# locuslab/lcp-physics

Hardware: AMD Instinct MI355X
Metric: sim steps/sec at batch=4096x16 contacts, fwd+bwd (higher is better)
Workload: dtype f64; 1 GPU; configs[2]: batch=4096 x 16 contacts (4-box stack, 4 pts/interface; nz 15, nineq 64, neq 3) per GPU, fp32 I/O, LCP forward + backward (implicit diff), mode=fused, bwd=dense; step outputs: new_v and the moved pose (engines.py:76-77, bodies.py:80-82), multipliers kept in the workspace in fp64; launch=eager: one ctypes call per kernel launch, device_spin_up_steps=4100, nonzero_status=0, global_batch=4096, parallelism=scenes sharded x1, no collectives, control_plane=single process

## Files before the change

lcp_physics_amd/csrc/lcp_quad_kernels.inc:

```
#pragma once
#include "lcp_quad_prims.h"

#ifndef LCP_Q_LAUNDER_IN_PLACE
#define LCP_Q_LAUNDER_IN_PLACE 1
#endif
#ifndef LCP_Q_PEEL_INIT
#define LCP_Q_PEEL_INIT 1
#endif
#ifndef LCP_Q_UNROLL_PASS
#define LCP_Q_UNROLL_PASS 1
#endif
#ifndef LCP_Q_NT_STORES
#define LCP_Q_NT_STORES 0
#endif
#ifndef LCP_Q_EXP_SPW
#define LCP_Q_EXP_SPW 4
#endif
#ifndef LCP_Q_RCP_STEP
#define LCP_Q_RCP_STEP 1
#endif
#ifndef LCP_Q_STEP_FAST
#define LCP_Q_STEP_FAST 1
#endif
#ifndef LCP_Q_OCC2
#define LCP_Q_OCC2 1
#endif
#ifndef LCP_Q_ROWL
#define LCP_Q_ROWL 0
#endif
#ifndef LCP_Q_BEST_LDS
#define LCP_Q_BEST_LDS 1
#endif

namespace lcp {
namespace q16 {

template <typename TI, typename TC>
struct LdsQ {
  TI* GL;
  TI* GTL;
  TI* AtL;
  TC* GAL;
  TC* S11;
// ... 331 lines not shown
  oz = m4<TC>(-wz.n, -wz.f1, -wz.f2, -wz.g);
  if (!valid) oz = m4<TC>(0, 0, 0, 0);
  os = m4<TC>((-rs.n - oz.n) * di.n, (-rs.f1 - oz.f1) * di.f1, (-rs.f2 - oz.f2) * di.f2, (-rs.g - oz.g) * di.g);
  if (!valid) os = m4<TC>(0, 0, 0, 0);
  oy = dy;
  const XV<TC, XH> gw = S.Gtw(oz.n, oz.f1 - oz.f2);
  XV<TC, XH> g1;
  static_for<XH>([&](auto HX) LCP_INL { g1.v[HX] = -rx.v[HX] - gw.v[HX]; });
  if (S.e > 0) { const XV<TC, XH> ay = S.Aty(dy); static_for<XH>([&](auto HX) LCP_INL { g1.v[HX] -= ay.v[HX]; }); }
  static_for<XH>([&](auto HX) LCP_INL { ox.v[HX] = S.qid[HX] * g1.v[HX]; });
  LCP_QTICK(pr, 5)
}

template <typename TC, bool PINC = false, int NZF = 0, int EF = 0, int NCF = 0>
struct PrimQ {
  static constexpr int NZF_ = NZF, EF_ = EF, NCF_ = NCF;
  static constexpr bool TRIM_ = PINC && NZF > 0;
  static constexpr int CLO_ = TRIM_ ? EF : 0, CHI_ = TRIM_ ? NZF : 16;
  TC idn, i1, i2, kap;
  TC udx, ude;
  bool pin_rt;
  __device__ __forceinline__ bool pin() const { return PINC || pin_rt; }
  TC sp[EQ];
};
template <typename TI, typename TC, typename PQ, typename SQ>
__device__ __forceinline__ M4<TC> minv_pq(const PQ& R, const SQ& S, const M4<TC>& t) {
  M4<TC> o;
  o.n = R.idn * t.n;
  o.g = R.kap * ((t.g - S.mu * o.n) + fma(R.i1, t.f1, R.i2 * t.f2));
  o.f1 = R.i1 * (t.f1 - o.g);
  o.f2 = R.i2 * (t.f2 - o.g);
  return o;
}
template <typename TI, typename TC, typename PQ, typename SQ>
__device__ __forceinline__ bool factor_pq(TC (&xr)[20], TC (&er)[20], PQ& R, const SQ& S, const M4<TC>& D,
                                          bool valid LCP_QPROF_ARG) {
  const int l16 = launder(S.l16), ncw = PQ::NCF_ > 0 ? PQ::NCF_ : __builtin_amdgcn_readfirstlane(S.ncw);
  const int nz = PQ::NZF_ > 0 ? PQ::NZF_ : __builtin_amdgcn_readfirstlane(S.nz), e = PQ::NZF_ > 0 ? PQ::EF_ : __builtin_amdgcn_readfirstlane(S.e);
  R.idn = fast_rcp(D.n); R.i1 = fast_rcp(D.f1); R.i2 = fast_rcp(D.f2);
  R.kap = fast_rcp(D.g + (R.i1 + R.i2));
  const TC b00 = valid ? R.idn : (TC)0;
  const TC b10 = valid ? R.kap * (R.i1 - R.i2) * (S.mu * R.idn) : (TC)0;
  const TC b11 = valid ? R.kap * fma(R.i1 + R.i2, D.g, (TC)4 * (R.i1 * R.i2)) : (TC)0;
  TC p0[16], p1[16];
  const int oz = lds_opaque_zero();
  constexpr int CLO = PQ::CLO_, CHI = PQ::CHI_;
  static_for<CHI - CLO>([&](auto Jq) LCP_INL {
    constexpr int J = CLO + Jq;
    const TC c = (TC)S.template jcv<J>(oz), t = (TC)S.template jtv<J>(oz); p0[J] = b00 * c; p1[J] = fma(b10, c, b11 * t);
  });
  {
    const TI* at = S.L.AtL + oz;
    const TC dsel = (l16 < nz) ? S.qd[0] : (TC)1;
    static_for<CHI - CLO>([&](auto Jq) LCP_INL { constexpr int J = CLO + Jq; xr[J] = (l16 == J) ? dsel : (TC)0; });
    if (!R.pin()) {
      static_for<16>([&](auto J) LCP_INL { er[J] = (l16 < EQ) ? (TC)at[(l16 & (EQ - 1)) * 16 + J] : (TC)0; });
      static_for<EQ>([&](auto A) LCP_INL {
        xr[16 + A] = (TC)at[A * 16 + l16];
        er[16 + A] = (l16 == A && A >= e) ? (TC)1 : (TC)0;
      });
    }
  }
  {
    const TI* gl = S.L.GL + l16 + oz;
    const TI* gtl = S.L.GTL + l16 + oz;
    static_for<2>([&](auto Hh) LCP_INL {
      constexpr int C0 = 8 * Hh;
      if (C0 < ncw) {
        TI gv[8], tv[8];
        if constexpr (sizeof(S.gcol) == sizeof(TC)) {
          static_for<8>([&](auto I) LCP_INL { gv[I] = gl[(C0 + I) * 16]; tv[I] = gtl[(C0 + I) * 16]; });
          __builtin_amdgcn_sched_barrier(0);
        }
        static_for<8>([&](auto I) LCP_INL {
          constexpr int C = C0 + I;
          TC a, b;
          if constexpr (sizeof(S.gcol) == sizeof(TC)) { a = (TC)gv[I]; b = (TC)tv[I]; } else { a = S.gcol[C]; b = S.tcol[C]; }
          if constexpr (PQ::TRIM_) {
            constexpr int NA = (CHI < 8 ? CHI : 8) - CLO, NB = CHI > 8 ? CHI - 8 : 0;
            pq_formN<C, CLO, (NA > 0 ? NA : 0)>(xr, p0, p1, a, b);
            pq_formN<C, 8, NB>(xr, p0, p1, a, b);
          } else {
            pq_form8<C, 0>(xr, p0, p1, a, b);
            pq_form8<C, 8>(xr, p0, p1, a, b);
          }
        });
      }
    });
  }
  LCP_QTICK(pr, 1)
  bool singular = false;
  R.udx = 1; R.ude = 1;
  if (R.pin()) {
    TC pivv = bc<0>(xr[0]);
    TC inv = (TC)1;
    bool primed = false;
    static_for<16>([&](auto K) LCP_INL {
      constexpr int k = K;
      if (k >= e && k < nz) {
        if (!primed) { pivv = bc<k>(xr[k]); inv = fast_rcp(pivv); primed = true; }
        singular = singular || (pivv == (TC)0);
        const TC sk = xr[k] * inv;
        const TC lx = keep_if(sk, l16 > k);
        xr[k] = (l16 == k) ? xr[k] : sk;
        R.udx = (l16 == k) ? inv : R.udx;
        if constexpr (k + 1 < 16) {
          fnmac_bc<k>(xr[k + 1], xr[k + 1], lx);
          pivv = bc<(k + 1) & 15>(xr[k + 1]); inv = fast_rcp(pivv);
          lu_cols_x<k, k + 2, 14 - k>(xr, lx);
        }
      }
    });
    if constexpr (!PQ::TRIM_)
      static_for<EQ>([&](auto A_) LCP_INL { constexpr int a = A_; R.sp[a] = xr[a]; xr[a] = (a < e) ? (TC)0 : xr[a]; });
    LCP_QTICK(pr, 2)
    return singular;
  }
  TC pivv = bc<0>(xr[0]);
  TC inv = fast_rcp(pivv);
  static_for<16>([&](auto K) LCP_INL {
    constexpr int k = K;
    if (k < nz) {
      singular = singular || (pivv == (TC)0);
      const TC lx = (l16 > k) ? xr[k] * inv : (TC)0;
      const TC le = er[k] * inv;
      xr[k] = (l16 > k) ? lx : xr[k];
      er[k] = le;
      R.udx = (l16 == k) ? inv : R.udx;
      fnmac_bc<k>(er[k + 1], xr[k + 1], le);
      fnmac_bc<k>(xr[k + 1], xr[k + 1], lx);
      if constexpr (k + 1 < 16) { pivv = bc<(k + 1) & 15>(xr[k + 1]); inv = fast_rcp(pivv); }
      lu_cols_p<k, k + 2, 18 - k>(xr, er, lx, le);
    }
  });
  static_for<EQ>([&](auto A_) LCP_INL {
    constexpr int a = A_, k = 16 + A_;
    if (a < e) {
      const TC pivv = bc<a>(er[k]);
      singular = singular || (pivv == (TC)0);
      const TC inv = fast_rcp(pivv);
      const TC le = (l16 > a) ? er[k] * inv : (TC)0;
      er[k] = (l16 > a) ? le : er[k];
      R.ude = (l16 == a) ? inv : R.ude;
      static_for<EQ - 1 - a>([&](auto JJ) LCP_INL { constexpr int j = k + 1 + JJ; fnmac_bc<a>(er[j], er[j], le); });
    }
  });
  LCP_QTICK(pr, 2)
  return singular;
}

template <typename TI, typename TC, typename PQ, typename SQ>
__device__ __forceinline__ void solve_kkt_pq(const SQ& S, const TC (&xr)[20], const TC (&er)[20], const PQ& R,
                                             const M4<TC>& di, bool valid, const XV<TC, 1>& rx, const M4<TC>& rs, const M4<TC>& rz, TC ry,
                                             XV<TC, 1>& ox, M4<TC>& os, M4<TC>& oz, TC& oy LCP_QPROF_ARG) {
  const int l16 = S.l16;
  const int nz = PQ::NZF_ > 0 ? PQ::NZF_ : __builtin_amdgcn_readfirstlane(S.nz), e = PQ::NZF_ > 0 ? PQ::EF_ : __builtin_amdgcn_readfirstlane(S.e);
  M4<TC> q = m4<TC>(rs.n * di.n - rz.n, rs.f1 * di.f1 - rz.f1, rs.f2 * di.f2 - rz.f2, rs.g * di.g - rz.g);
  if (!valid) q = m4<TC>(0, 0, 0, 0);
  const M4<TC> u = minv_pq<TI, TC, PQ, SQ>(R, S, q);
  const XV<TC, 1> gu = S.template Gtw<true>(valid ? u.n : (TC)0, valid ? u.f1 - u.f2 : (TC)0);
  TC wx = (l16 < nz) ? gu.v[0] - rx.v[0] : (TC)0;
  TC we = (l16 < e) ? -ry : (TC)0;
  LCP_QTICK(pr, 3)
  if (R.pin()) {
    if constexpr (PQ::TRIM_) {
      static_for<PQ::CHI_ - PQ::CLO_>([&](auto Kq) LCP_INL { constexpr int k = PQ::CLO_ + Kq; fnmac_bc<k>(wx, wx, keep_if(xr[k], l16 > k)); });
      static_for<PQ::CHI_ - PQ::CLO_>([&](auto KR) LCP_INL { constexpr int k = PQ::CHI_ - 1 - KR; fnmac_bc<k>(wx, wx, keep_if(xr[k], l16 < k)); });
    } else {
    if (e > 0) static_for<EQ>([&](auto A_) LCP_INL { constexpr int a = A_; fnmac_bc<a>(wx, we, keep_if(R.sp[a], a < e)); });
    static_for<4>([&](auto Gq) LCP_INL {
      if (4 * Gq < nz) static_for<4>([&](auto Kq) LCP_INL {
        constexpr int k = 4 * Gq + Kq;
        fnmac_bc<k>(wx, wx, keep_if(xr[k], l16 > k));
      });
    });
    static_for<4>([&](auto GR) LCP_INL {
      constexpr int Gq = 3 - GR;
      if (4 * Gq < nz) static_for<4>([&](auto KR) LCP_INL {
        constexpr int k = 4 * Gq + 3 - KR;
        fnmac_bc<k>(wx, wx, keep_if(xr[k], l16 < k));
      });
    });
    }
    LCP_QTICK(pr, 4)
    ox.v[0] = (l16 < e) ? we : ((l16 < nz) ? wx * R.udx : (TC)0);
    oy = (l16 < e) ? wx : (TC)0;
    TC gn, gt;
    S.template Gv<true, PQ::CLO_, PQ::CHI_>(ox, gn, gt);
    oz = minv_pq<TI, TC, PQ, SQ>(R, S, m4<TC>(gn - q.n, gt - q.f1, -gt - q.f2, -q.g));
    if (!valid) oz = m4<TC>(0, 0, 0, 0);
    os = m4<TC>((-rs.n - oz.n) * di.n, (-rs.f1 - oz.f1) * di.f1, (-rs.f2 - oz.f2) * di.f2, (-rs.g - oz.g) * di.g);
    if (!valid) os = m4<TC>(0, 0, 0, 0);
    LCP_QTICK(pr, 5)
    return;
  }
  static_for<4>([&](auto Gq) LCP_INL {
    if (4 * Gq < nz) static_for<4>([&](auto Kq) LCP_INL {
      constexpr int k = 4 * Gq + Kq;
      fnmac_bc<k>(we, wx, er[k]);
      fnmac_bc<k>(wx, wx, keep_if(xr[k], l16 > k));
    });
  });
  if (e > 0) {
    static_for<EQ>([&](auto A_) LCP_INL { constexpr int a = A_; fnmac_bc<a>(we, we, keep_if(er[16 + a], l16 > a)); });
    static_for<EQ>([&](auto AR) LCP_INL {
      constexpr int a = EQ - 1 - AR;
      const TC xs = we * R.ude;
      fnmac_bc<a>(wx, xs, xr[16 + a]);
      fnmac_bc<a>(we, xs, keep_if(er[16 + a], l16 < a));
    });
  }
  static_for<4>([&](auto GR) LCP_INL {
    constexpr int Gq = 3 - GR;
    if (4 * Gq < nz) static_for<4>([&](auto KR) LCP_INL {
      constexpr int k = 4 * Gq + 3 - KR;
      const TC xs = wx * R.udx;
      fnmac_bc<k>(wx, xs, keep_if(xr[k], l16 < k));
    });
  });
  LCP_QTICK(pr, 4)
  ox.v[0] = (l16 < nz) ? wx * R.udx : (TC)0;
  oy = (l16 < e) ? we * R.ude : (TC)0;
  TC gn, gt;
  S.template Gv<true>(ox, gn, gt);
  oz = minv_pq<TI, TC, PQ, SQ>(R, S, m4<TC>(gn - q.n, gt - q.f1, -gt - q.f2, -q.g));
  if (!valid) oz = m4<TC>(0, 0, 0, 0);
  os = m4<TC>((-rs.n - oz.n) * di.n, (-rs.f1 - oz.f1) * di.f1, (-rs.f2 - oz.f2) * di.f2, (-rs.g - oz.g) * di.g);
  if (!valid) os = m4<TC>(0, 0, 0, 0);
  LCP_QTICK(pr, 5)
}

template <typename TC>
__device__ __forceinline__ TC step_pair_q(const M4<TC>& z, const M4<TC>& dz, const M4<TC>& s, const M4<TC>& ds, bool valid) {
  const TC ninf = -inf_of<TC>(), pinf = inf_of<TC>();
  const M4<TC> az = m4<TC>(qdiv_x(-z.n, dz.n), qdiv_x(-z.f1, dz.f1), qdiv_x(-z.f2, dz.f2), qdiv_x(-z.g, dz.g));
  const M4<TC> as = m4<TC>(qdiv_x(-s.n, ds.n), qdiv_x(-s.f1, ds.f1), qdiv_x(-s.f2, ds.f2), qdiv_x(-s.g, ds.g));
  auto key4 = [&](const M4<TC>& a) { return umax(umax(nan_key(a.n), nan_key(a.f1)), umax(nan_key(a.f2), nan_key(a.g))); };
#if LCP_Q_STEP_FAST
  {
    const bool oz = !(dz.n > (TC)0) || !(dz.f1 > (TC)0) || !(dz.f2 > (TC)0) || !(dz.g > (TC)0);
    const bool os = !(ds.n > (TC)0) || !(ds.f1 > (TC)0) || !(ds.f2 > (TC)0) || !(ds.g > (TC)0);
    const bool nn = key_is_nan<TC>(umax(key4(az), key4(as)));
    uint32_t f = valid ? (8u | (oz ? 1u : 0u) | (os ? 2u : 0u) | (nn ? 4u : 0u)) : 0u;
    f |= (uint32_t)__builtin_amdgcn_update_dpp(0, (int)f, 0xB1, 0xf, 0xf, true);
    f |= (uint32_t)__builtin_amdgcn_update_dpp(0, (int)f, 0x4E, 0xf, 0xf, true);
    f |= (uint32_t)__builtin_amdgcn_update_dpp(0, (int)f, 0x141, 0xf, 0xf, true);
    f |= (uint32_t)__builtin_amdgcn_update_dpp(0, (int)f, 0x140, 0xf, 0xf, true);
    if (__all(f == 11u || f == 0u)) {
      auto open = [&](TC dv, TC a) { return (dv > (TC)0) ? pinf : a; };
      TC l = fmin_(fmin_(fmin_(open(dz.n, az.n), open(dz.f1, az.f1)), fmin_(open(dz.f2, az.f2), open(dz.g, az.g))),
                   fmin_(fmin_(open(ds.n, as.n), open(ds.f1, as.f1)), fmin_(open(ds.f2, as.f2), open(ds.g, as.g))));
      return row_fmin(valid ? l : pinf);
    }
  }
#endif
  TC mz = valid ? fmax_(fmax_(az.n, az.f1), fmax_(az.f2, az.g)) : ninf;
  TC ms = valid ? fmax_(fmax_(as.n, as.f1), fmax_(as.f2, as.g)) : ninf;
  const uint32_t kmz = row_umax(valid ? key4(az) : 0u), kms = row_umax(valid ? key4(as) : 0u);
  mz = row_fmax(mz); ms = row_fmax(ms);
  const TC fz = key_is_nan<TC>(kmz) ? (TC)1 : fmax_(mz, (TC)1), fs = key_is_nan<TC>(kms) ? (TC)1 : fmax_(ms, (TC)1);
  auto pick = [&](TC dv, TC a, TC fill) { return (dv > (TC)0) ? fill : a; };
  const M4<TC> pz = m4<TC>(pick(dz.n, az.n, fz), pick(dz.f1, az.f1, fz), pick(dz.f2, az.f2, fz), pick(dz.g, az.g, fz));
// ... 386 lines not shown
      rx = S.template Gtw<ALG != 0>(z.n, z.f1 - z.f2);
      static_for<XH>([&](auto HX) LCP_INL { rx.v[HX] = rx.v[HX] + S.qd[HX] * x.v[HX] + p.v[HX]; });
      if (e > 0) {
        if constexpr (ALG != 0) {
          if (R.pin()) rx.v[0] += (l16 < e) ? y : (TC)0;
          else { const XVt ay_ = S.Aty(y); rx.v[0] += ay_.v[0]; }
        } else { const XVt ay_ = S.Aty(y); static_for<XH>([&](auto HX) LCP_INL { rx.v[HX] += ay_.v[HX]; }); }
      }
      rs = POST ? m4<TC>(z.n, 0, 0, 0) : z;
      TC gn, gt;
      constexpr int GLO = (ALG == 2 && NZF > 0) ? EF : 0, GHI = (ALG == 2 && NZF > 0) ? NZF : 16;
      S.template Gv<ALG != 0, GLO, GHI>(x, gn, gt);
      rz = POST ? m4<TC>(gn + s.n - hn, 0, 0, 0) : m4<TC>(gn + s.n - hn, gt + s.f1 - z.g, -gt + s.f2 - z.g, s.g - (S.mu * z.n - (z.f1 + z.f2)));
      if (!vc) rz = m4<TC>(0, 0, 0, 0);
      if constexpr (ALG != 0) ry = (e > 0) ? (R.pin() ? ((l16 < e) ? x.v[0] : (TC)0) : (S.Av(x) - b)) : (TC)0;
      else ry = (e > 0) ? (S.Av(x) - b) : (TC)0;
      TC rx2 = 0;
      static_for<XH>([&](auto HX) LCP_INL { rx2 += (16 * HX + l16 < nz) ? rx.v[HX] * rx.v[HX] : (TC)0; });
      const TC n_rx = row_sum(rx2);
      const TC n_rz = row_sum(rz.n * rz.n + rz.f1 * rz.f1 + rz.f2 * rz.f2 + rz.g * rz.g);
      TC n_ry = 0;
      if constexpr (!(ALG == 2 && NZF > 0)) n_ry = row_sum((l16 < e) ? ry * ry : (TC)0);
      const TC sz = row_sum(vc ? (POST ? s.n * z.n : (s.n * z.n + s.f1 * z.f1) + (s.f2 * z.f2 + s.g * z.g)) : (TC)0);
      szsum = sz;
      mu = sz / mf; mu = mu < 0 ? -mu : mu;
      resid = sqrt(n_rz) + sqrt(n_ry) + sqrt(n_rx) + mf * mu;
      if constexpr (POST) dinv = vc ? m4<TC>(s.n * fast_rcp(z.n), 1, 1, 1) : m4<TC>(1, 1, 1, 1);
      else if constexpr (RCPS) dinv = vc ? m4<TC>(s.n * fast_rcp(z.n), s.f1 * fast_rcp(z.f1), s.f2 * fast_rcp(z.f2), s.g * fast_rcp(z.g)) : m4<TC>(1, 1, 1, 1);
      else
      dinv = vc ? m4<TC>(qdiv(s.n, z.n), qdiv(s.f1, z.f1), qdiv(s.f2, z.f2), qdiv(s.g, z.g)) : m4<TC>(1, 1, 1, 1);
    }
    LCP_QTICK(pr, 0)
    bool sing_;
    if constexpr (ALG == 0) sing_ = factor_q<TI, TC, LCP_Q_LDSW != 0, XH>(ta, tu, R, S, W.R2, dinv, vc LCP_QPROF_PASS);
    else sing_ = factor_pq<TI, TC, decltype(R)>(ta, tu, R, S, dinv, vc LCP_QPROF_PASS);
    const bool singular = row_any(sing_);
    if (ALG != 0 && it < 0 && singular && e > 0) status |= LCP_ST_SINGULAR_S11;
    if (it >= 0 && !done) {
      ++iters;
      if (singular && it > 0) { status |= LCP_ST_SINGULAR_T; done = true; }
      else {
        const bool improved = !have_best || (resid < best_resid);
        if (improved) {
          best_resid = resid; n_not = 0; have_best = true;
          if constexpr (BEST_LDS) park(x, y, z, s); else { bx = x; by = y; bz = z; bs = s; }
        } else ++n_not;
        if (n_not == lim || best_resid < eps || mu > mu_limit<TC>()) done = true;
      }
    }
    if (!__any(!done)) LCP_Q_BREAK;
    if (it >= 0 && it == max_iter - 1) LCP_Q_BREAK;
    LCP_QTICK(pr, 6)
    XVt ax;
    static_for<XH>([&](auto HX) LCP_INL { ax.v[HX] = 0; });
    TC ay = 0;
    M4<TC> as_ = m4<TC>(0, 0, 0, 0), az = as_;
    const int npass = (it < 0) ? 1 : 2;
#if LCP_Q_UNROLL_PASS
    auto one_pass = [&](auto PASS_) LCP_INL {
      constexpr int pass = PASS_;
#else
#pragma unroll 1
    for (int pass = 0; pass < npass; ++pass) {
#endif
      XVt ox;
      TC oy;
      M4<TC> os, oz;
      if constexpr (ALG == 0) solve_kkt_q<TI, TC, XH>(S, ta, tu, R, dinv, vc, rx, rs, rz, ry, ox, os, oz, oy, pass == 1 LCP_QPROF_PASS);
      else solve_kkt_pq<TI, TC, decltype(R)>(S, ta, tu, R, dinv, vc, rx, rs, rz, ry, ox, os, oz, oy LCP_QPROF_PASS);
      if (it < 0) {
        x = ox; s = os; z = oz; y = oy;
        if constexpr (POST) { s = m4<TC>(s.n, 1, 1, 1); z = m4<TC>(z.n, 1, 1, 1); }
        const TC smin = row_pmin(vc ? (POST ? s.n : pmin(pmin(s.n, s.f1), pmin(s.f2, s.g))) : inf_of<TC>());
        const TC zmin = row_pmin(vc ? (POST ? z.n : pmin(pmin(z.n, z.f1), pmin(z.f2, z.g))) : inf_of<TC>());
        if (smin <= (TC)0) { const TC sh = (TC)1 - smin; s = m4<TC>(s.n + sh, s.f1 + sh, s.f2 + sh, s.g + sh); }
        if (zmin <= (TC)0) { const TC sh = (TC)1 - zmin; z = m4<TC>(z.n + sh, z.f1 + sh, z.f2 + sh, z.g + sh); }
        if (!vc) { s = m4<TC>(1, 1, 1, 1); z = s; }
        if constexpr (POST) { s = m4<TC>(s.n, 1, 1, 1); z = m4<TC>(z.n, 1, 1, 1); }
        if (ncs == 0 && !done) {
          if constexpr (BEST_LDS) { bestL[0] = x.v[0]; bestL[64] = y; } else { bx = x; by = y; }
          done = true;
        }
      } else if (pass == 0) {
        ax = ox; ay = oy; as_ = os; az = oz;
        if constexpr (BEST_LDS) {
          stashL[0] = ax.v[0]; stashL[64] = ay;
          stashL[128] = as_.n; stashL[192] = as_.f1; stashL[256] = as_.f2; stashL[320] = as_.g;
          stashL[384] = az.n; stashL[448] = az.f1; stashL[512] = az.f2; stashL[576] = az.g;
        }
        M4<TC> irs = m4<TC>(1, 1, 1, 1), irz = irs;
        if constexpr (POST) { irs = m4<TC>(fast_rcp(s.n), 1, 1, 1); irz = m4<TC>(dinv.n * irs.n, 1, 1, 1); }
        else if constexpr (RCPS) {
          irs = m4<TC>(fast_rcp(s.n), fast_rcp(s.f1), fast_rcp(s.f2), fast_rcp(s.g));
          irz = m4<TC>(dinv.n * irs.n, dinv.f1 * irs.f1, dinv.f2 * irs.f2, dinv.g * irs.g);
        }
        TC alpha;
        if constexpr (POST) alpha = pmin(step_pair_rcp<true>(irz, az, irs, as_, vc), (TC)1);
        else if constexpr (RCPS) alpha = pmin(step_pair_rcp(irz, az, irs, as_, vc), (TC)1);
        else alpha = pmin(step_pair_q(z, az, s, as_, vc), (TC)1);
        auto sc = [&](TC sv, TC dsv, TC zv, TC dzv) { return (sv + alpha * dsv) * (zv + alpha * dzv); };
        const TC t3 = row_sum(vc ? (POST ? sc(s.n, as_.n, z.n, az.n) : (sc(s.n, as_.n, z.n, az.n) + sc(s.f1, as_.f1, z.f1, az.f1)) + (sc(s.f2, as_.f2, z.f2, az.f2) + sc(s.g, as_.g, z.g, az.g))) : (TC)0);
// ... 158 lines not shown
  if (vc && row_any(sing)) { dinv.n = fmax_(dinv.n, fa); dinv.f1 = fmax_(dinv.f1, fu); dinv.f2 = fmax_(dinv.f2, fu); }
  factor_q<TI, TC, false, XH>(ta, tu, R, S, W2q, dinv, vc LCP_QPROF_PASS);
}

#ifndef LCP_Q_BWD_FLOOR
#define LCP_Q_BWD_FLOOR 1e-12
#endif
#ifndef LCP_Q_BWD_ONE_SOLVE
#define LCP_Q_BWD_ONE_SOLVE 0
#endif
#ifndef LCP_Q_BWD_REFINE
#define LCP_Q_BWD_REFINE 1
#endif
template <typename TI, typename TC, int NZF = 0, int EF = 0, bool PINB = false>
__device__ __forceinline__ void bwd_solve_body(const SceneQ<TI, TC, 1>& S, bool vc, const M4<TC>& z, const M4<TC>& s, TC g,
                                               TC& dx, M4<TC>& dl, TC& dnu LCP_QPROF_ARG) {
  const int l16 = S.l16, nz = NZF > 0 ? NZF : S.nz, e = NZF > 0 ? EF : S.e;
  using PQb = PrimQ<TC, PINB, NZF, EF>;
  const M4<TC> dinv = vc ? m4<TC>(s.n / z.n, s.f1 / z.f1, s.f2 / z.f2, s.g / z.g) : m4<TC>(1, 1, 1, 1);
  M4<TC> dfl = dinv;
  {
    TC wn = 0, wt = 0;
    static_for<16>([&](auto J) LCP_INL { const TC qi = bc<J>(S.qid[0]); wn = fma((TC)S.jc[J] * (TC)S.jc[J], qi, wn); wt = fma((TC)S.jt[J] * (TC)S.jt[J], qi, wt); });
    constexpr TC BWD_FLOOR = (TC)LCP_Q_BWD_FLOOR;
    if (vc) { dfl.n = fmax_(dinv.n, BWD_FLOOR * wn); dfl.f1 = fmax_(dinv.f1, BWD_FLOOR * wt); dfl.f2 = fmax_(dinv.f2, BWD_FLOOR * wt); }
  }
  PQb R;
  {
    bool okl = true;
    static_for<EQ>([&](auto A_) LCP_INL { constexpr int a = A_; if (a < e) okl = okl && ((TC)S.L.AtL[a * 16 + l16] == ((l16 == a) ? (TC)1 : (TC)0)); });
    R.pin_rt = PINB ? true : (__all(okl) != 0);
  }
  TC xr[20], er[20];
  factor_pq<TI, TC, PQb>(xr, er, R, S, dfl, vc LCP_QPROF_PASS);
  const M4<TC> zero = m4<TC>(0, 0, 0, 0);
  XV<TC, 1> rx, ox;
#if LCP_Q_BWD_ONE_SOLVE
  dx = 0; dnu = 0; dl = zero;
  int passes = 1 + LCP_Q_BWD_REFINE; asm volatile("" : "+s"(passes));
#pragma unroll 1
  for (int ref = 0; ref < passes; ++ref) {
#else
  M4<TC> ds;
  rx.v[0] = g;
  solve_kkt_pq<TI, TC, PQb>(S, xr, er, R, dfl, vc, rx, zero, zero, (TC)0, ox, ds, dl, dnu LCP_QPROF_PASS);
  dx = ox.v[0];
#pragma unroll 1
  for (int ref = 0; ref < LCP_Q_BWD_REFINE; ++ref) {
#endif
    const XV<TC, 1> gl = S.template Gtw<false>(vc ? dl.n : (TC)0, vc ? dl.f1 - dl.f2 : (TC)0);
    TC r1 = -g - (S.qd[0] * dx + gl.v[0]);
    if (e > 0) { const XV<TC, 1> ay = S.Aty(dnu); r1 -= ay.v[0]; }
    if (!(l16 < nz)) r1 = 0;
    TC gn, gt;
    ox.v[0] = dx;
    S.template Gv<false>(ox, gn, gt);
    M4<TC> r3 = m4<TC>(-(gn - dinv.n * dl.n), -(gt - (dinv.f1 * dl.f1 + dl.g)), -(-gt - (dinv.f2 * dl.f2 + dl.g)),
                       (S.mu * dl.n - (dl.f1 + dl.f2)) + dinv.g * dl.g);
    if (!vc) r3 = zero;
    const TC r2 = (e > 0) ? -S.Av(ox) : (TC)0;
    XV<TC, 1> cx;
    M4<TC> cs, cl;
    TC cnu;
    rx.v[0] = -r1;
    solve_kkt_pq<TI, TC, PQb>(S, xr, er, R, dfl, vc, rx, zero, m4<TC>(-r3.n, -r3.f1, -r3.f2, -r3.g), -r2, cx, cs, cl, cnu LCP_QPROF_PASS);
    dx += cx.v[0]; dnu += cnu;
    dl = m4<TC>(dl.n + cl.n, dl.f1 + cl.f1, dl.f2 + cl.f2, dl.g + cl.g);
  }
}

template <typename TI, typename TC, bool BODY = false, int NZF = 0, int EF = 0, bool PINB = false>
__global__ void __launch_bounds__(64) lcp_bwd_quad(BwdArgs P, int lds_per_scene, int accept) {
  static_assert(NZF == 0 || BODY, "compile-time sizes: the body-space backward");
  extern __shared__ __attribute__((aligned(16))) unsigned char smem_all[];
  const int lane = threadIdx.x, l16 = lane & 15, row = lane >> 4;
  const int scene_raw = blockIdx.x * 4 + row;
  const int scene = scene_raw < P.B ? scene_raw : P.B - 1;
  const int nz = NZF > 0 ? NZF : P.nz, nc = P.m >> 2, e = NZF > 0 ? EF : P.e, m = P.m;
// ... 344 lines not shown
```

lcp_physics_amd/csrc/lcp_quad_prims.h:

```cpp
#pragma once
#include "lcp_wave_common.h"

namespace lcp {
namespace q16 {

using namespace w64;

constexpr int NCQ = 16;
constexpr int EQ = 4;

template <int K> __device__ __forceinline__ float bc(float v) {
  return __builtin_bit_cast(float, __builtin_amdgcn_update_dpp(0, __builtin_bit_cast(int, v), 0x150 + K, 0xf, 0xf, true));
}
template <int K> __device__ __forceinline__ double bc(double v) {
  return __builtin_amdgcn_update_dpp(0.0, v, 0x150 + K, 0xf, 0xf, true);
}
template <int K, typename T> __device__ __forceinline__ void fmac_bc(T& acc, T src, T mult) { acc = fma(bc<K>(src), mult, acc); }
template <int K, typename T> __device__ __forceinline__ void fnmac_bc(T& acc, T src, T mult) { acc = fma(bc<K>(src), -mult, acc); }
#ifndef LCP_Q_ASM_LU
#define LCP_Q_ASM_LU 1
#endif
#ifndef LCP_Q_TS_GROUP
#define LCP_Q_TS_GROUP 4
#endif
// ... 242 lines not shown
}

template <int K, int J0, int N> struct LuColsP;
#define LCP_LUP_DEF(N)                                                                                                   \
  template <int K, int J0> struct LuColsP<K, J0, N> {                                                                    \
    static __device__ __forceinline__ void run(double (&ta)[20], double (&tu)[20], double la, double lu) {               \
      asm("s_nop 1\n\t" LCP_LUA_S##N : LCP_LUA_O##N : [la] "v"(la), [lu] "v"(lu), [k] "n"(K));                           \
    }                                                                                                                    \
  };
LCP_LUP_DEF(1) LCP_LUP_DEF(2) LCP_LUP_DEF(3) LCP_LUP_DEF(4) LCP_LUP_DEF(5) LCP_LUP_DEF(6) LCP_LUP_DEF(7)
LCP_LUP_DEF(8) LCP_LUP_DEF(9) LCP_LUP_DEF(10) LCP_LUP_DEF(11) LCP_LUP_DEF(12) LCP_LUP_DEF(13) LCP_LUP_DEF(14)
template <int K, int J0, int N> __device__ __forceinline__ void lu_cols_p(double (&xr)[20], double (&er)[20], double lx, double le) {
  if constexpr (N > 14) { LuColsP<K, J0, 14>::run(xr, er, lx, le); lu_cols_p<K, J0 + 14, N - 14>(xr, er, lx, le); }
  else if constexpr (N > 0) LuColsP<K, J0, N>::run(xr, er, lx, le);
}
template <int K, int J0, int N> __device__ __forceinline__ void lu_cols_p(float (&xr)[20], float (&er)[20], float lx, float le) {
  static_for<N>([&](auto JJ) LCP_INL { constexpr int j = J0 + JJ; const float sj = bc<K>(xr[j]); er[j] = fmaf(-le, sj, er[j]); xr[j] = fmaf(-lx, sj, xr[j]); });
}
template <int K, int J0, int N> struct LuColsX;
#define LCP_LUX_DEF(N)                                                                                                   \
  template <int K, int J0> struct LuColsX<K, J0, N> {                                                                    \
    static __device__ __forceinline__ void run(double (&tu)[20], double lu) {                                            \
      asm("s_nop 1\n\t" LCP_LUU_S##N : LCP_LUU_O##N : [lu] "v"(lu), [k] "n"(K));                                         \
    }                                                                                                                    \
  };
LCP_LUX_DEF(1) LCP_LUX_DEF(2) LCP_LUX_DEF(3) LCP_LUX_DEF(4) LCP_LUX_DEF(5) LCP_LUX_DEF(6) LCP_LUX_DEF(7)
LCP_LUX_DEF(8) LCP_LUX_DEF(9) LCP_LUX_DEF(10) LCP_LUX_DEF(11) LCP_LUX_DEF(12) LCP_LUX_DEF(13) LCP_LUX_DEF(14)
template <int K, int J0, int N> __device__ __forceinline__ void lu_cols_x(double (&xr)[20], double lx) {
  if constexpr (N > 0) LuColsX<K, J0, N>::run(xr, lx);
}
template <int K, int J0, int N> __device__ __forceinline__ void lu_cols_x(float (&xr)[20], float lx) {
  static_for<N>([&](auto JJ) LCP_INL { constexpr int j = J0 + JJ; xr[j] = fmaf(-lx, bc<K>(xr[j]), xr[j]); });
}
#define LCP_PQF_ONE(X, P, M) "v_fmac_f64_dpp %[" #X "], %[" #P "], %[" #M "] row_newbcast:%[k] " LCP_DPP_FULL "\n\t"
template <int K, int J0> __device__ __forceinline__ void pq_form8(double (&xr)[20], const double (&p0)[16], const double (&p1)[16], double a, double b) {
  asm("s_nop 1\n\t" LCP_PQF_ONE(x0, p0, a) LCP_PQF_ONE(x1, p1, a) LCP_PQF_ONE(x2, p2, a) LCP_PQF_ONE(x3, p3, a) LCP_PQF_ONE(x4, p4, a) LCP_PQF_ONE(x5, p5, a) LCP_PQF_ONE(x6, p6, a) LCP_PQF_ONE(x7, p7, a) LCP_PQF_ONE(x0, q0, b) LCP_PQF_ONE(x1, q1, b) LCP_PQF_ONE(x2, q2, b) LCP_PQF_ONE(x3, q3, b) LCP_PQF_ONE(x4, q4, b) LCP_PQF_ONE(x5, q5, b) LCP_PQF_ONE(x6, q6, b) LCP_PQF_ONE(x7, q7, b)
      : [x0] "+v"(xr[J0 + 0]), [x1] "+v"(xr[J0 + 1]), [x2] "+v"(xr[J0 + 2]), [x3] "+v"(xr[J0 + 3]), [x4] "+v"(xr[J0 + 4]), [x5] "+v"(xr[J0 + 5]), [x6] "+v"(xr[J0 + 6]), [x7] "+v"(xr[J0 + 7])
      : [p0] "v"(p0[J0 + 0]), [q0] "v"(p1[J0 + 0]), [p1] "v"(p0[J0 + 1]), [q1] "v"(p1[J0 + 1]), [p2] "v"(p0[J0 + 2]), [q2] "v"(p1[J0 + 2]), [p3] "v"(p0[J0 + 3]), [q3] "v"(p1[J0 + 3]), [p4] "v"(p0[J0 + 4]), [q4] "v"(p1[J0 + 4]), [p5] "v"(p0[J0 + 5]), [q5] "v"(p1[J0 + 5]), [p6] "v"(p0[J0 + 6]), [q6] "v"(p1[J0 + 6]), [p7] "v"(p0[J0 + 7]), [q7] "v"(p1[J0 + 7]), [a] "v"(a), [b] "v"(b), [k] "n"(K));
}
template <int K, int J0> __device__ __forceinline__ void pq_form8(float (&xr)[20], const float (&p0)[16], const float (&p1)[16], float a, float b) {
  static_for<8>([&](auto JJ) LCP_INL { constexpr int j = J0 + JJ; xr[j] = fmaf(bc<K>(p0[j]), a, xr[j]); xr[j] = fmaf(bc<K>(p1[j]), b, xr[j]); });
}

#ifndef LCP_DPP_FULL_EARLY
#define LCP_DPP_FULL_EARLY "row_mask:0xf bank_mask:0xf"
#endif
#ifndef LCP_GV_ONE
#define LCP_GV_ONE(ACC, M, K) "v_fmac_f64_dpp %[" #ACC "], %[v], %[" #M "] row_newbcast:%[" #K "] " LCP_DPP_FULL_EARLY "\n\t"
#endif
template <int K, int J0, int N> struct PqFormN;
template <int J0, int N> struct GvN;
template <int K, int J0> struct PqFormN<K, J0, 1> { static __device__ __forceinline__ void run(double (&xr)[20], const double (&p0)[16], const double (&p1)[16], double a, double b) {
  asm("s_nop 1\n\t" LCP_PQF_ONE(x0, p0, a) LCP_PQF_ONE(x0, q0, b) 
      : [x0] "+v"(xr[J0 + 0])
      : [p0] "v"(p0[J0 + 0]), [q0] "v"(p1[J0 + 0]), [a] "v"(a), [b] "v"(b), [k] "n"(K)); } };
template <int K, int J0> struct PqFormN<K, J0, 2> { static __device__ __forceinline__ void run(double (&xr)[20], const double (&p0)[16], const double (&p1)[16], double a, double b) {
  asm("s_nop 1\n\t" LCP_PQF_ONE(x0, p0, a) LCP_PQF_ONE(x1, p1, a) LCP_PQF_ONE(x0, q0, b) LCP_PQF_ONE(x1, q1, b) 
      : [x0] "+v"(xr[J0 + 0]), [x1] "+v"(xr[J0 + 1])
      : [p0] "v"(p0[J0 + 0]), [q0] "v"(p1[J0 + 0]), [p1] "v"(p0[J0 + 1]), [q1] "v"(p1[J0 + 1]), [a] "v"(a), [b] "v"(b), [k] "n"(K)); } };
template <int K, int J0> struct PqFormN<K, J0, 3> { static __device__ __forceinline__ void run(double (&xr)[20], const double (&p0)[16], const double (&p1)[16], double a, double b) {
  asm("s_nop 1\n\t" LCP_PQF_ONE(x0, p0, a) LCP_PQF_ONE(x1, p1, a) LCP_PQF_ONE(x2, p2, a) LCP_PQF_ONE(x0, q0, b) LCP_PQF_ONE(x1, q1, b) LCP_PQF_ONE(x2, q2, b) 
      : [x0] "+v"(xr[J0 + 0]), [x1] "+v"(xr[J0 + 1]), [x2] "+v"(xr[J0 + 2])
      : [p0] "v"(p0[J0 + 0]), [q0] "v"(p1[J0 + 0]), [p1] "v"(p0[J0 + 1]), [q1] "v"(p1[J0 + 1]), [p2] "v"(p0[J0 + 2]), [q2] "v"(p1[J0 + 2]), [a] "v"(a), [b] "v"(b), [k] "n"(K)); } };
template <int K, int J0> struct PqFormN<K, J0, 4> { static __device__ __forceinline__ void run(double (&xr)[20], const double (&p0)[16], const double (&p1)[16], double a, double b) {
  asm("s_nop 1\n\t" LCP_PQF_ONE(x0, p0, a) LCP_PQF_ONE(x1, p1, a) LCP_PQF_ONE(x2, p2, a) LCP_PQF_ONE(x3, p3, a) LCP_PQF_ONE(x0, q0, b) LCP_PQF_ONE(x1, q1, b) LCP_PQF_ONE(x2, q2, b) LCP_PQF_ONE(x3, q3, b) 
      : [x0] "+v"(xr[J0 + 0]), [x1] "+v"(xr[J0 + 1]), [x2] "+v"(xr[J0 + 2]), [x3] "+v"(xr[J0 + 3])
// ... 59 lines not shown
```

Before: 56.37 million sim steps/s.

## Fold forward substitution of first solve RHS into pinned LU factorization

The right-hand side for the first KKT solve is now computed before factorization, and its forward-elimination sweep is fused into the pinned LU column updates through a new inline-asm helper that also updates the RHS register. Later, the solve's forward pass is skipped for that pass, in both the forward iterations and the backward implicit-diff solve. This removes a separate dependent chain of DPP broadcast FMAs per solve. The cost is a longer factorization asm block, extra live registers for q, wx and we, and a more tangled control flow with special cases for the last iteration and the trimmed (TRIM) layout.

New measurement: 55.69 million sim steps/s. -1.2%, worse.

```diff
diff --git a/lcp_physics_amd/csrc/lcp_quad_kernels.inc b/lcp_physics_amd/csrc/lcp_quad_kernels.inc
--- a/lcp_physics_amd/csrc/lcp_quad_kernels.inc
+++ b/lcp_physics_amd/csrc/lcp_quad_kernels.inc
@@ -9,6 +9,9 @@
 #endif
 #ifndef LCP_Q_UNROLL_PASS
 #define LCP_Q_UNROLL_PASS 1
+#endif
+#ifndef LCP_Q_RHS_IN_LU
+#define LCP_Q_RHS_IN_LU 1
 #endif
 #ifndef LCP_Q_NT_STORES
 #define LCP_Q_NT_STORES 0
@@ -406,13 +409,30 @@
   o.f2 = R.i2 * (t.f2 - o.g);
   return o;
 }
+template <typename TC, typename PQ>
+__device__ __forceinline__ void minv_rcps_pq(PQ& R, const M4<TC>& D) {
+  R.idn = fast_rcp(D.n); R.i1 = fast_rcp(D.f1); R.i2 = fast_rcp(D.f2);
+  R.kap = fast_rcp(D.g + (R.i1 + R.i2));
+}
 template <typename TI, typename TC, typename PQ, typename SQ>
+__device__ __forceinline__ void rhs_pq(const SQ& S, const PQ& R, const M4<TC>& di, bool valid, const XV<TC, 1>& rx, const M4<TC>& rs,
+                                       const M4<TC>& rz, TC ry, M4<TC>& q, TC& wx, TC& we LCP_QPROF_ARG) {
+  const int l16 = S.l16;
+  const int nz = PQ::NZF_ > 0 ? PQ::NZF_ : __builtin_amdgcn_readfirstlane(S.nz), e = PQ::NZF_ > 0 ? PQ::EF_ : __builtin_amdgcn_readfirstlane(S.e);
+  q = m4<TC>(rs.n * di.n - rz.n, rs.f1 * di.f1 - rz.f1, rs.f2 * di.f2 - rz.f2, rs.g * di.g - rz.g);
+  if (!valid) q = m4<TC>(0, 0, 0, 0);
+  const M4<TC> u = minv_pq<TI, TC, PQ, SQ>(R, S, q);
+  const XV<TC, 1> gu = S.template Gtw<true>(valid ? u.n : (TC)0, valid ? u.f1 - u.f2 : (TC)0);
+  wx = (l16 < nz) ? gu.v[0] - rx.v[0] : (TC)0;
+  we = (l16 < e) ? -ry : (TC)0;
+  LCP_QTICK(pr, 3)
+}
+template <typename TI, typename TC, typename PQ, bool AUG = false, typename SQ>
 __device__ __forceinline__ bool factor_pq(TC (&xr)[20], TC (&er)[20], PQ& R, const SQ& S, const M4<TC>& D,
-                                          bool valid LCP_QPROF_ARG) {
+                                          bool valid, TC& wx, TC we LCP_QPROF_ARG) {
   const int l16 = launder(S.l16), ncw = PQ::NCF_ > 0 ? PQ::NCF_ : __builtin_amdgcn_readfirstlane(S.ncw);
   const int nz = PQ::NZF_ > 0 ? PQ::NZF_ : __builtin_amdgcn_readfirstlane(S.nz), e = PQ::NZF_ > 0 ? PQ::EF_ : __builtin_amdgcn_readfirstlane(S.e);
-  R.idn = fast_rcp(D.n); R.i1 = fast_rcp(D.f1); R.i2 = fast_rcp(D.f2);
-  R.kap = fast_rcp(D.g + (R.i1 + R.i2));
+  if constexpr (!AUG) minv_rcps_pq<TC, PQ>(R, D);
   const TC b00 = valid ? R.idn : (TC)0;
   const TC b10 = valid ? R.kap * (R.i1 - R.i2) * (S.mu * R.idn) : (TC)0;
   const TC b11 = valid ? R.kap * fma(R.i1 + R.i2, D.g, (TC)4 * (R.i1 * R.i2)) : (TC)0;
@@ -469,6 +489,10 @@
     TC pivv = bc<0>(xr[0]);
     TC inv = (TC)1;
     bool primed = false;
+    if constexpr (AUG && !PQ::TRIM_) {
+      if (e > 0) static_for<EQ>([&](auto A_) LCP_INL { constexpr int a = A_; fnmac_bc<a>(wx, we, keep_if(xr[a], a < e)); });
+      static_for<EQ>([&](auto A_) LCP_INL { constexpr int a = A_; if (a < e) fnmac_bc<a>(wx, wx, (TC)0); });
+    }
     static_for<16>([&](auto K) LCP_INL {
       constexpr int k = K;
       if (k >= e && k < nz) {
@@ -481,8 +505,9 @@
         if constexpr (k + 1 < 16) {
           fnmac_bc<k>(xr[k + 1], xr[k + 1], lx);
           pivv = bc<(k + 1) & 15>(xr[k + 1]); inv = fast_rcp(pivv);
-          lu_cols_x<k, k + 2, 14 - k>(xr, lx);
-        }
+          if constexpr (AUG) lu_cols_xw<k, k + 2, 14 - k>(xr, wx, lx);
+          else lu_cols_x<k, k + 2, 14 - k>(xr, lx);
+        } else if constexpr (AUG) fnmac_bc<k>(wx, wx, lx);
       }
     });
     if constexpr (!PQ::TRIM_)
@@ -524,23 +549,24 @@
 }
 
 template <typename TI, typename TC, typename PQ, typename SQ>
-__device__ __forceinline__ void solve_kkt_pq(const SQ& S, const TC (&xr)[20], const TC (&er)[20], const PQ& R,
-                                             const M4<TC>& di, bool valid, const XV<TC, 1>& rx, const M4<TC>& rs, const M4<TC>& rz, TC ry,
-                                             XV<TC, 1>& ox, M4<TC>& os, M4<TC>& oz, TC& oy LCP_QPROF_ARG) {
+__device__ __forceinline__ bool factor_pq(TC (&xr)[20], TC (&er)[20], PQ& R, const SQ& S, const M4<TC>& D, bool valid LCP_QPROF_ARG) {
+  TC wx = 0;
+  return factor_pq<TI, TC, PQ, false>(xr, er, R, S, D, valid, wx, (TC)0 LCP_QPROF_PASS);
+}
+
+template <typename TI, typename TC, typename PQ, bool FOLDED, typename SQ>
+__device__ __forceinline__ void sweep_pq(const SQ& S, const TC (&xr)[20], const TC (&er)[20], const PQ& R, const M4<TC>& di, bool valid,
+                                         const M4<TC>& q, TC wx, TC we, const M4<TC>& rs,
+                                         XV<TC, 1>& ox, M4<TC>& os, M4<TC>& oz, TC& oy LCP_QPROF_ARG) {
   const int l16 = S.l16;
   const int nz = PQ::NZF_ > 0 ? PQ::NZF_ : __builtin_amdgcn_readfirstlane(S.nz), e = PQ::NZF_ > 0 ? PQ::EF_ : __builtin_amdgcn_readfirstlane(S.e);
-  M4<TC> q = m4<TC>(rs.n * di.n - rz.n, rs.f1 * di.f1 - rz.f1, rs.f2 * di.f2 - rz.f2, rs.g * di.g - rz.g);
-  if (!valid) q = m4<TC>(0, 0, 0, 0);
-  const M4<TC> u = minv_pq<TI, TC, PQ, SQ>(R, S, q);
-  const XV<TC, 1> gu = S.template Gtw<true>(valid ? u.n : (TC)0, valid ? u.f1 - u.f2 : (TC)0);
-  TC wx = (l16 < nz) ? gu.v[0] - rx.v[0] : (TC)0;
-  TC we = (l16 < e) ? -ry : (TC)0;
-  LCP_QTICK(pr, 3)
   if (R.pin()) {
     if constexpr (PQ::TRIM_) {
+      if constexpr (!FOLDED)
       static_for<PQ::CHI_ - PQ::CLO_>([&](auto Kq) LCP_INL { constexpr int k = PQ::CLO_ + Kq; fnmac_bc<k>(wx, wx, keep_if(xr[k], l16 > k)); });
       static_for<PQ::CHI_ - PQ::CLO_>([&](auto KR) LCP_INL { constexpr int k = PQ::CHI_ - 1 - KR; fnmac_bc<k>(wx, wx, keep_if(xr[k], l16 < k)); });
     } else {
+    if constexpr (!FOLDED) {
     if (e > 0) static_for<EQ>([&](auto A_) LCP_INL { constexpr int a = A_; fnmac_bc<a>(wx, we, keep_if(R.sp[a], a < e)); });
     static_for<4>([&](auto Gq) LCP_INL {
       if (4 * Gq < nz) static_for<4>([&](auto Kq) LCP_INL {
@@ -548,6 +574,7 @@
         fnmac_bc<k>(wx, wx, keep_if(xr[k], l16 > k));
       });
     });
+    }
     static_for<4>([&](auto GR) LCP_INL {
       constexpr int Gq = 3 - GR;
       if (4 * Gq < nz) static_for<4>([&](auto KR) LCP_INL {
@@ -602,6 +629,15 @@
   os = m4<TC>((-rs.n - oz.n) * di.n, (-rs.f1 - oz.f1) * di.f1, (-rs.f2 - oz.f2) * di.f2, (-rs.g - oz.g) * di.g);
   if (!valid) os = m4<TC>(0, 0, 0, 0);
   LCP_QTICK(pr, 5)
+}
+template <typename TI, typename TC, typename PQ, typename SQ>
+__device__ __forceinline__ void solve_kkt_pq(const SQ& S, const TC (&xr)[20], const TC (&er)[20], const PQ& R,
+                                             const M4<TC>& di, bool valid, const XV<TC, 1>& rx, const M4<TC>& rs, const M4<TC>& rz, TC ry,
+                                             XV<TC, 1>& ox, M4<TC>& os, M4<TC>& oz, TC& oy LCP_QPROF_ARG) {
+  M4<TC> q;
+  TC wx, we;
+  rhs_pq<TI, TC, PQ>(S, R, di, valid, rx, rs, rz, ry, q, wx, we LCP_QPROF_PASS);
+  sweep_pq<TI, TC, PQ, false>(S, xr, er, R, di, valid, q, wx, we, rs, ox, os, oz, oy LCP_QPROF_PASS);
 }
 
 template <typename TC>
@@ -1054,8 +1090,18 @@
     }
     LCP_QTICK(pr, 0)
     bool sing_;
+    [[maybe_unused]] M4<TC> q0 = m4<TC>(0, 0, 0, 0);
+    [[maybe_unused]] TC wx0 = 0, we0 = 0;
     if constexpr (ALG == 0) sing_ = factor_q<TI, TC, LCP_Q_LDSW != 0, XH>(ta, tu, R, S, W.R2, dinv, vc LCP_QPROF_PASS);
+#if LCP_Q_RHS_IN_LU
+    else {
+      minv_rcps_pq<TC>(R, dinv);
+      if (!(it >= 0 && it == max_iter - 1)) rhs_pq<TI, TC, decltype(R)>(S, R, dinv, vc, rx, rs, rz, ry, q0, wx0, we0 LCP_QPROF_PASS);
+      sing_ = factor_pq<TI, TC, decltype(R), true>(ta, tu, R, S, dinv, vc, wx0, we0 LCP_QPROF_PASS);
+    }
+#else
     else sing_ = factor_pq<TI, TC, decltype(R)>(ta, tu, R, S, dinv, vc LCP_QPROF_PASS);
+#endif
     const bool singular = row_any(sing_);
     if (ALG != 0 && it < 0 && singular && e > 0) status |= LCP_ST_SINGULAR_S11;
     if (it >= 0 && !done) {
@@ -1089,6 +1135,9 @@
       TC oy;
       M4<TC> os, oz;
       if constexpr (ALG == 0) solve_kkt_q<TI, TC, XH>(S, ta, tu, R, dinv, vc, rx, rs, rz, ry, ox, os, oz, oy, pass == 1 LCP_QPROF_PASS);
+#if LCP_Q_RHS_IN_LU
+      else if (pass == 0) sweep_pq<TI, TC, decltype(R), true>(S, ta, tu, R, dinv, vc, q0, wx0, we0, rs, ox, os, oz, oy LCP_QPROF_PASS);
+#endif
       else solve_kkt_pq<TI, TC, decltype(R)>(S, ta, tu, R, dinv, vc, rx, rs, rz, ry, ox, os, oz, oy LCP_QPROF_PASS);
       if (it < 0) {
         x = ox; s = os; z = oz; y = oy;
@@ -1313,9 +1362,18 @@
     R.pin_rt = PINB ? true : (__all(okl) != 0);
   }
   TC xr[20], er[20];
-  factor_pq<TI, TC, PQb>(xr, er, R, S, dfl, vc LCP_QPROF_PASS);
   const M4<TC> zero = m4<TC>(0, 0, 0, 0);
   XV<TC, 1> rx, ox;
+#if LCP_Q_RHS_IN_LU && !LCP_Q_BWD_ONE_SOLVE
+  M4<TC> q0;
+  TC wx0, we0;
+  rx.v[0] = g;
+  minv_rcps_pq<TC>(R, dfl);
+  rhs_pq<TI, TC, PQb>(S, R, dfl, vc, rx, zero, zero, (TC)0, q0, wx0, we0 LCP_QPROF_PASS);
+  factor_pq<TI, TC, PQb, true>(xr, er, R, S, dfl, vc, wx0, we0 LCP_QPROF_PASS);
+#else
+  factor_pq<TI, TC, PQb>(xr, er, R, S, dfl, vc LCP_QPROF_PASS);
+#endif
 #if LCP_Q_BWD_ONE_SOLVE
   dx = 0; dnu = 0; dl = zero;
   int passes = 1 + LCP_Q_BWD_REFINE; asm volatile("" : "+s"(passes));
@@ -1323,8 +1381,12 @@
   for (int ref = 0; ref < passes; ++ref) {
 #else
   M4<TC> ds;
+#if LCP_Q_RHS_IN_LU
+  sweep_pq<TI, TC, PQb, true>(S, xr, er, R, dfl, vc, q0, wx0, we0, zero, ox, ds, dl, dnu LCP_QPROF_PASS);
+#else
   rx.v[0] = g;
   solve_kkt_pq<TI, TC, PQb>(S, xr, er, R, dfl, vc, rx, zero, zero, (TC)0, ox, ds, dl, dnu LCP_QPROF_PASS);
+#endif
   dx = ox.v[0];
 #pragma unroll 1
   for (int ref = 0; ref < LCP_Q_BWD_REFINE; ++ref) {
diff --git a/lcp_physics_amd/csrc/lcp_quad_prims.h b/lcp_physics_amd/csrc/lcp_quad_prims.h
--- a/lcp_physics_amd/csrc/lcp_quad_prims.h
+++ b/lcp_physics_amd/csrc/lcp_quad_prims.h
@@ -298,6 +298,23 @@
 template <int K, int J0, int N> __device__ __forceinline__ void lu_cols_x(float (&xr)[20], float lx) {
   static_for<N>([&](auto JJ) LCP_INL { constexpr int j = J0 + JJ; xr[j] = fmaf(-lx, bc<K>(xr[j]), xr[j]); });
 }
+template <int K, int J0, int N> struct LuColsXW;
+#define LCP_LUXW_DEF(N)                                                                                                  \
+  template <int K, int J0> struct LuColsXW<K, J0, N> {                                                                   \
+    static __device__ __forceinline__ void run(double (&tu)[20], double& w, double lu) {                                 \
+      asm("s_nop 1\n\t" LCP_LUU_S##N LCP_LUU_COL(w) : LCP_LUU_O##N , [w] "+v"(w) : [lu] "v"(lu), [k] "n"(K));            \
+    }                                                                                                                    \
+  };
+LCP_LUXW_DEF(1) LCP_LUXW_DEF(2) LCP_LUXW_DEF(3) LCP_LUXW_DEF(4) LCP_LUXW_DEF(5) LCP_LUXW_DEF(6) LCP_LUXW_DEF(7)
+LCP_LUXW_DEF(8) LCP_LUXW_DEF(9) LCP_LUXW_DEF(10) LCP_LUXW_DEF(11) LCP_LUXW_DEF(12) LCP_LUXW_DEF(13) LCP_LUXW_DEF(14)
+template <int K, int J0, int N> __device__ __forceinline__ void lu_cols_xw(double (&xr)[20], double& w, double lx) {
+  if constexpr (N > 0) LuColsXW<K, J0, N>::run(xr, w, lx);
+  else fnmac_bc<K>(w, w, lx);
+}
+template <int K, int J0, int N> __device__ __forceinline__ void lu_cols_xw(float (&xr)[20], float& w, float lx) {
+  lu_cols_x<K, J0, N>(xr, lx);
+  fnmac_bc<K>(w, w, lx);
+}
 #define LCP_PQF_ONE(X, P, M) "v_fmac_f64_dpp %[" #X "], %[" #P "], %[" #M "] row_newbcast:%[k] " LCP_DPP_FULL "\n\t"
 template <int K, int J0> __device__ __forceinline__ void pq_form8(double (&xr)[20], const double (&p0)[16], const double (&p1)[16], double a, double b) {
   asm("s_nop 1\n\t" LCP_PQF_ONE(x0, p0, a) LCP_PQF_ONE(x1, p1, a) LCP_PQF_ONE(x2, p2, a) LCP_PQF_ONE(x3, p3, a) LCP_PQF_ONE(x4, p4, a) LCP_PQF_ONE(x5, p5, a) LCP_PQF_ONE(x6, p6, a) LCP_PQF_ONE(x7, p7, a) LCP_PQF_ONE(x0, q0, b) LCP_PQF_ONE(x1, q1, b) LCP_PQF_ONE(x2, q2, b) LCP_PQF_ONE(x3, q3, b) LCP_PQF_ONE(x4, q4, b) LCP_PQF_ONE(x5, q5, b) LCP_PQF_ONE(x6, q6, b) LCP_PQF_ONE(x7, q7, b)
```
